# fluggo/Canvas

Hardware: AMD Instinct MI355X
Metric: Mpixels/s through 4K f16 RGBA colour-matrix+alpha-over chain; % HBM roofline (higher is better)
Workload: dtype f32

## Files before the change

### canvas_amd/csrc/host/color.c

```c
#include "internal.h"

CVS_EXPORT int cvs_color_matrix_f16_dev(rgba_frame_f16 *frame, const float m[9], int pre_lut, int post_lut, cvs_stream_t s) {
    if (cvs_enter() != 0) return -1;
    CVS_REQUIRE_INSIDE(frame, frame, "cvs_color_matrix_f16_dev");
    if (box2i_is_empty(&frame->current_window)) return 0;
    if (!cvs_box_contains(&frame->full_window, &frame->current_window)) { cvs_set_error("colour matrix: current_window outside the buffer"); return -1; }
    const half *pre = cvs_lut_dev_or_null(pre_lut), *post = cvs_lut_dev_or_null(post_lut);
    if ((pre_lut != CVS_LUT_NONE && !pre) || (post_lut != CVS_LUT_NONE && !post)) return -1;
    cvk_view v = cvs_view(frame->data, &frame->full_window);
    CVS_KERNEL(CVK(cvk_color_matrix)(v, v, cvs_rect(&frame->current_window), m, pre, post, cvs_cus(), cvs_pick_stream(s)));
    return 0;
}

CVS_EXPORT int cvs_color_matrix_f16_to_dev(rgba_frame_f16 *out, const rgba_frame_f16 *in, const float m[9], int pre_lut, int post_lut, cvs_stream_t s) {
    if (cvs_enter() != 0) { box2i_set_empty(&out->current_window); return -1; }
    CVS_REQUIRE_INSIDE(in, out, "cvs_color_matrix_f16_to_dev");
    box2i win;
    box2i_intersect(&win, &out->full_window, &in->current_window);
    out->current_window = win;
    if (box2i_is_empty(&win)) return 0;
    if (!cvs_box_contains(&in->full_window, &win)) { cvs_set_error("colour matrix: source window outside its buffer"); box2i_set_empty(&out->current_window); return -1; }
    const half *pre = cvs_lut_dev_or_null(pre_lut), *post = cvs_lut_dev_or_null(post_lut);
    if ((pre_lut != CVS_LUT_NONE && !pre) || (post_lut != CVS_LUT_NONE && !post)) { box2i_set_empty(&out->current_window); return -1; }
    CVS_KERNEL(CVK(cvk_color_matrix)(cvs_view(out->data, &out->full_window), cvs_view(in->data, &in->full_window), cvs_rect(&win), m, pre, post, cvs_cus(), cvs_pick_stream(s)));
    return 0;
}

static void host_color(rgba_frame_f16 *frame, const float m[9], int pre, int post) {
    if (box2i_is_empty(&frame->current_window) || cvs_enter() != 0) return;
    hipStream_t s = cvs_pick_stream(NULL);
    cvs_staged d = { 0 };
    rgba_frame_f16 f = *frame;
    int rc = cvs_stage_in(&d, frame->data, cvs_box_pixels(&frame->full_window) * sizeof(rgba_f16), 1, s);
    f.data = d.dev;
    if (rc == 0) rc = cvs_color_matrix_f16_dev(&f, m, pre, post, s);
    if (rc == 0) cvs_stage_out(&d, frame->data, s);
    cvs_stage_free(&d);
}

CVS_EXPORT void video_color_rgb_to_xyz_sdtv(rgba_frame_f16 *frame) {
    static const float m[9] = { 0.3936f, 0.2124f, 0.0187f, 0.3652f, 0.7010f, 0.1119f, 0.1916f, 0.0865f, 0.9582f };
    host_color(frame, m, CVS_LUT_REC709_TO_LINEAR_SCENE, CVS_LUT_NONE);
}

CVS_EXPORT void video_color_xyz_to_srgb(rgba_frame_f16 *frame) {
    static const float m[9] = { 3.2410f, -0.9692f, 0.0556f, -1.5374f, 1.8760f, -0.2040f, -0.4986f, 0.0416f, 1.0570f };
    host_color(frame, m, CVS_LUT_NONE, CVS_LUT_LINEAR_TO_SRGB);
}


static __thread int t_last_fused = -1;
CVS_EXPORT int cvs_chain_last_was_fused(void) { return t_last_fused; }
CVS_EXPORT int cvs_chain_last_launch_count(void) { return CVK(cvk_chain_count)(); }

static bool same_box(const box2i *a, const box2i *b) {
    return a->min.x == b->min.x && a->min.y == b->min.y && a->max.x == b->max.x && a->max.y == b->max.y;
}

static bool ranges_overlap(const void *a, const void *b, size_t bytes) {
    const uintptr_t x = (uintptr_t)a, y = (uintptr_t)b;
    return x < y + bytes && y < x + bytes;
}

static bool job_is_fusable(const cvs_chain_job *j) {
    if (j->nlayers < 1 || j->nlayers > CVS_CHAIN_MAX_LAYERS) return false;
    const box2i *fw = &j->out->full_window;
    if (box2i_is_empty(fw) || cvs_box_pixels(fw) < 2) return false;
    if (((uintptr_t)j->out->data & 15u) != 0) return false;
    const size_t bytes = cvs_box_pixels(fw) * sizeof(rgba_f16);
    for (int k = 0; k < j->nlayers; k++) {
        const rgba_frame_f16 *l = j->layers[k];
        if (!same_box(&l->full_window, fw) || !same_box(&l->current_window, fw)) return false;
        if (((uintptr_t)l->data & 15u) != 0) return false;
        if (l->data != j->out->data && ranges_overlap(l->data, j->out->data, bytes)) return false;
    }
    return true;
}

static bool job_depends_on_earlier(const cvs_chain_job *jobs, int first, int j) {
    const size_t bj = cvs_box_pixels(&jobs[j].out->full_window) * sizeof(rgba_f16);
    for (int i = first; i < j; i++) {
        const size_t bi = cvs_box_pixels(&jobs[i].out->full_window) * sizeof(rgba_f16);
        const size_t span = bi > bj ? bi : bj;
        if (ranges_overlap(jobs[j].out->data, jobs[i].out->data, span)) return true;
// ... 37 lines not shown

CVS_EXPORT int cvs_chain_color_over_f16_dev(const cvs_chain_job *jobs, int njobs, const float m[9],
                                            int pre_lut, int post_lut, cvs_stream_t stream) {
    if (cvs_enter() != 0) return -1;
    if (njobs <= 0) return 0;
    hipStream_t s = cvs_pick_stream(stream);
    if (!m && (pre_lut != CVS_LUT_NONE || post_lut != CVS_LUT_NONE)) { cvs_set_error("chain: transfer tables need a colour matrix (m == NULL means no colour stage)"); return -1; }
    const half *pre = cvs_lut_dev_or_null(pre_lut), *post = cvs_lut_dev_or_null(post_lut);
    if ((pre_lut != CVS_LUT_NONE && !pre) || (post_lut != CVS_LUT_NONE && !post)) return -1;

    bool all_fusable = true;
    for (int i = 0; i < njobs; i++) all_fusable = all_fusable && job_is_fusable(&jobs[i]);
    if (!all_fusable) {
        t_last_fused = 0;
        for (int i = 0; i < njobs; i++) {
            int rc = chain_unfused(&jobs[i], m, pre_lut, post_lut, s);
            if (rc != 0) return rc;
        }
        return 0;
    }

    cvk_chain_job *recs = calloc((size_t)njobs, sizeof *recs);
    if (!recs) { cvs_set_error("chain: out of host memory"); return -1; }
    int uniform = jobs[0].nlayers;
    for (int i = 0; i < njobs; i++) {
        cvk_chain_job *kj = &recs[i];
        kj->out = jobs[i].out->data;
        for (int k = 0; k < jobs[i].nlayers; k++) kj->layer[k] = jobs[i].layers[k]->data;
        kj->nlayers = jobs[i].nlayers;
        kj->npixels = cvs_box_pixels(&jobs[i].out->full_window);
        if (jobs[i].nlayers != uniform) uniform = 0;
        jobs[i].out->current_window = jobs[i].out->full_window;
    }
    int rc = 0;
    CVK(cvk_chain_count_reset)();
    for (int first = 0; rc == 0 && first < njobs; ) {
        int end = first + 1;
        while (end < njobs && !job_depends_on_earlier(jobs, first, end)) end++;
        rc = CVK(cvk_chain_color_over)(recs + first, end - first, uniform, m, pre, post, cvs_cus(), s);
        first = end;
    }
    free(recs);
    if (rc != 0) { cvs_set_error("chain kernel launch failed: %s", hipGetErrorString((hipError_t)rc)); return rc; }
    t_last_fused = 1;
    return 0;
}

CVS_EXPORT int cvs_mix_cross_f16_dev(rgba_frame_f16 *out, const rgba_frame_f16 *a, const rgba_frame_f16 *b, float mix_b, cvs_stream_t stream) {
    if (cvs_enter() != 0) { box2i_set_empty(&out->current_window); return -1; }
    CVS_REQUIRE_INSIDE(a, out, "cvs_mix_cross_f16_dev");
    CVS_REQUIRE_INSIDE(b, out, "cvs_mix_cross_f16_dev");
    hipStream_t s = cvs_pick_stream(stream);
    mix_b = clampf(mix_b, 0.0f, 1.0f);
    const cvs_chain_job job = { out, { a, b }, 2 };
    if (job_is_fusable(&job)) {
        cvk_chain_job rec;
        memset(&rec, 0, sizeof rec);
        rec.out = out->data; rec.layer[0] = a->data; rec.layer[1] = b->data; rec.nlayers = 2;
        rec.npixels = cvs_box_pixels(&out->full_window);
        int rc = CVK(cvk_chain_cross)(&rec, 1, 1.0f - mix_b, mix_b, cvs_cus(), s);
        if (rc != 0) { cvs_set_error("crossfade kernel launch failed: %s", hipGetErrorString((hipError_t)rc)); box2i_set_empty(&out->current_window); return rc; }
        out->current_window = out->full_window;
        t_last_fused = 1;
        return 0;
    }
    t_last_fused = 0;
    const box2i *fw = &out->full_window;
    const size_t n = cvs_box_pixels(fw);
    if (!n) { box2i_set_empty(&out->current_window); return 0; }
    rgba_frame_f32 fa = { cvs_pool_malloc(n * sizeof(rgba_f32), s), *fw, *fw }, fb = { cvs_pool_malloc(n * sizeof(rgba_f32), s), *fw, *fw };
    rgba_frame_f32 fo = { cvs_pool_malloc(n * sizeof(rgba_f32), s), *fw, *fw };
    int rc = (fa.data && fb.data && fo.data) ? 0 : -1;
    rgba_frame_f16 clip = { cvs_pool_malloc(n * sizeof(rgba_f16), s), *fw, *fw };
    if (!clip.data) rc = -1;
    if (rc == 0) rc = cvs_copy_frame_f16_dev(&clip, a, s);
    if (rc == 0) rc = cvs_frame_f16_to_f32_dev(&fa, &clip, s);
    if (rc == 0) rc = cvs_copy_frame_f16_dev(&clip, b, s);
    if (rc == 0) rc = cvs_frame_f16_to_f32_dev(&fb, &clip, s);
    if (rc == 0) rc = cvs_mix_cross_f32_dev(&fo, &fa, &fb, mix_b, s);
    if (rc == 0) rc = cvs_frame_f32_to_f16_dev(out, &fo, s);
    cvs_pool_free(clip.data, s); cvs_pool_free(fa.data, s); cvs_pool_free(fb.data, s); cvs_pool_free(fo.data, s);
    if (rc != 0) box2i_set_empty(&out->current_window);
    return rc;
}
```

### canvas_amd/csrc/kernels/chain_deep_ops.hip

```cpp
#include "chain_kernel.hpp"

namespace {

template <int NL, int DIAG>
int launch_mode(const BatchT<8> &b, int n, const Mat &mat, const uint16_t *pre, const uint16_t *post, unsigned grid, unsigned block, int lshift, hipStream_t s) {
    if (mat.plain) return launch<NL, CHAIN_PLAIN, DIAG>(b, n, mat, pre, post, grid, block, lshift, s);
    return launch<NL, CHAIN_GRADE, DIAG>(b, n, mat, pre, post, grid, block, lshift, s);
}

template <int DIAG>
int launch_deep(int nl, const BatchT<8> &b, int n, const Mat &mat, const uint16_t *pre, const uint16_t *post, unsigned grid, unsigned block, int lshift, hipStream_t s) {
    switch (nl) {
    case 5: return launch_mode<5, DIAG>(b, n, mat, pre, post, grid, block, lshift, s);
    case 6: return launch_mode<6, DIAG>(b, n, mat, pre, post, grid, block, lshift, s);
    case 7: return launch_mode<7, DIAG>(b, n, mat, pre, post, grid, block, lshift, s);
    default: return launch_mode<8, DIAG>(b, n, mat, pre, post, grid, block, lshift, s);
    }
}

}

extern "C" int cvk_chain_deep(const cvk_chain_job *jobs, int njobs, int nlayers, const cvs::Mat *mat, const uint16_t *pre, const uint16_t *post,
                              unsigned grid, unsigned block, int lshift, int diag, uint64_t bytes_per_launch, void *stream, int *taken) {
    if (nlayers < 5 || nlayers > 8 || mat->cross || block > 512) return (int)hipErrorInvalidValue;
    BatchT<8> b;
    const int n = fill_batch(b, jobs, njobs, nlayers, bytes_per_launch);
    *taken = n;
    hipStream_t s = (hipStream_t)stream;
#ifdef CVS_DIAG
    if (diag == DIAG_MEMORY_ONLY) return launch_deep<DIAG_MEMORY_ONLY>(nlayers, b, n, *mat, pre, post, grid, block, lshift, s);
    if (diag == DIAG_COMPUTE_ONLY) return launch_deep<DIAG_COMPUTE_ONLY>(nlayers, b, n, *mat, pre, post, grid, block, lshift, s);
#endif
    (void)diag;
    return launch_deep<DIAG_NONE>(nlayers, b, n, *mat, pre, post, grid, block, lshift, s);
}
```

### canvas_amd/csrc/kernels/chain_kernel.hpp

```cpp
#pragma once
#include "lut_common.hpp"
#include "grade.hpp"
#include "chain_math.hpp"
#include <string.h>

namespace {

using namespace cvs;

template <int ML> struct JobCT { void *out; const void *layer[ML]; uint64_t npixels; };
template <int ML> struct BatchT {
    static constexpr int kJobs = ML == 4 ? 64 : 48;
    JobCT<ML> jobs[kJobs];
};
template <int ML>
inline int fill_batch(BatchT<ML> &b, const cvk_chain_job *jobs, int njobs, int nlayers, uint64_t bytes_per_launch) {
    memset(&b, 0, sizeof b);
    uint64_t bytes = 0;
    int n = 0;
    while (n < njobs && n < BatchT<ML>::kJobs) {
        const cvk_chain_job &src = jobs[n];
        const uint64_t job_bytes = src.npixels * 8 * (uint64_t)(nlayers + 1);
        if (n > 0 && bytes + job_bytes > bytes_per_launch) break;
        b.jobs[n].out = src.out;
// ... 36 lines not shown

__device__ __forceinline__ void stage_lut_any(uint16_t *lds, const uint16_t *__restrict__ table) {
    const uint4 *src = reinterpret_cast<const uint4 *>(table);
    uint4 *dst = reinterpret_cast<uint4 *>(lds);
    constexpr int kWords = kLutHalfs * 2 / 16;
    if (kWords % blockDim.x == 0) {
        const int slices = kWords / (int)blockDim.x, rot = (int)(blockIdx.x >> 3);
        for (int it = 0; it < slices; it++) {
            const int i = ((it + rot) % slices) * (int)blockDim.x + (int)threadIdx.x;
            dst[i] = src[i];
        }
    } else {
        for (int i = threadIdx.x; i < kWords; i += blockDim.x) dst[i] = src[i];
    }
    __syncthreads();
}

enum { DIAG_NONE = 0, DIAG_MEMORY_ONLY = 1, DIAG_COMPUTE_ONLY = 2 };

template <int NL>
struct Walk {
    unsigned job;
    unsigned chunk;
    unsigned npairs;
    unsigned nchunks;
    const char *layer[NL];
    char *out;
};

constexpr bool chain_hand_pipelined(int nl, int mode, bool pre, bool post) {
    return !(nl == 6 && mode == CHAIN_GRADE && pre && !post);
}

template <int NL, int MODE, bool PRE, bool POST, int DIAG>
__global__ __launch_bounds__(NL <= 4 ? kWG : 512) void k_chain(BatchT<(NL <= 4 ? 4 : 8)> batch, int njobs_, Mat kmat, int lshift,
                                               const uint16_t *__restrict__ pre, const uint16_t *__restrict__ post) {
    constexpr bool HAND = chain_hand_pipelined(NL, MODE, PRE, POST);
    const MatR mat = CVS_MAT_REGS(kmat);
    __shared__ uint16_t lut[(PRE || POST) ? kLutHalfs : 1];
    const unsigned L = 1u << lshift, G = gridDim.x, tid = threadIdx.x, njobs = (unsigned)njobs_;

    auto load_job = [&](Walk<NL> &w) {
        const auto &job = batch.jobs[w.job];
        w.npairs = (unsigned)(job.npixels >> 1);
        w.nchunks = (w.npairs + L - 1) >> lshift;
#pragma unroll
        for (int k = 0; k < NL; k++) w.layer[k] = reinterpret_cast<const char *>(job.layer[k]);
        w.out = reinterpret_cast<char *>(job.out);
    };
    auto advance = [&](Walk<NL> &w, unsigned by) {
        w.chunk += by;
        while (w.chunk >= w.nchunks) {
            w.chunk -= w.nchunks;
            if (++w.job >= njobs) { w.job = njobs; w.chunk = 0; return; }
            load_job(w);
        }
    };
    auto valid_of = [&](const Walk<NL> &w) -> unsigned { const unsigned left = w.npairs - (w.chunk << lshift); return left < L ? left : L; };
    auto issue = [&](u32x4 (&dst)[NL], const Walk<NL> &w) {
        const unsigned valid = valid_of(w);
        const uint32_t voff = (tid < valid ? tid : valid - 1) << 4;
#pragma unroll
        for (int k = 0; k < NL; k++) {
            const char *base = w.layer[k] + ((size_t)w.chunk << (lshift + 4));
            if constexpr (HAND) asm_ld4s(dst[k], base, voff);
            else dst[k] = __builtin_nontemporal_load(reinterpret_cast<const u32x4 *>(base + voff));
        }
    };

    Walk<NL> cur;
    cur.job = 0; cur.chunk = 0;
    load_job(cur);
    advance(cur, blockIdx.x);
    if (cur.job >= njobs) return;
    Walk<NL> next = cur;
    advance(next, G);

    u32x4 A[NL], B[NL];
    u32x4 diag_acc = { 0, 0, 0, 0 };
    issue(A, cur);
    if (PRE) stage_lut_any(lut, pre);
    else if (POST) stage_lut_any(lut, post);
    if constexpr (HAND) wait_vm0(A);
    if (next.job < njobs) issue(B, next);

    auto trip = [&](u32x4 (&now)[NL], u32x4 (&nxt)[NL]) -> bool {
        u32x4 res;
        if (DIAG == DIAG_MEMORY_ONLY) {
            res = now[0];
#pragma unroll
            for (int k = 1; k < NL; k++) res ^= now[k];
        } else {
            res = chain_pair_lean<NL, PRE, POST, MODE>(now, mat, lut, post);
        }
        Walk<NL> after = next;
        if (after.job < njobs) advance(after, G);
        const bool store_it = tid < valid_of(cur);
        g_u4 out = (g_u4)(cur.out + ((size_t)cur.chunk << (lshift + 4)));
        __builtin_amdgcn_sched_barrier(0);
        if constexpr (HAND) wait_vm0(nxt);
        __builtin_amdgcn_sched_barrier(0);
        if (DIAG == DIAG_COMPUTE_ONLY) diag_acc ^= res;
        else if (store_it) __builtin_nontemporal_store(res, out + tid);
        if (after.job < njobs) {
            if (DIAG == DIAG_COMPUTE_ONLY) {
#pragma unroll
                for (int k = 0; k < NL; k++) now[k] = nxt[k];
            } else {
                issue(now, after);
            }
        }
        __builtin_amdgcn_sched_barrier(0);
        cur = next;
        next = after;
        return cur.job < njobs;
    };
    while (trip(A, B) && trip(B, A)) { }
    if (DIAG == DIAG_COMPUTE_ONLY) ((g_u4)batch.jobs[0].out)[(size_t)blockIdx.x * L + tid] = diag_acc;

}

template <int NL, int MODE, bool PRE, bool POST>
__global__ __launch_bounds__(64) void k_chain_tail(BatchT<(NL <= 4 ? 4 : 8)> batch, int njobs, Mat kmat, const uint16_t *__restrict__ pre, const uint16_t *__restrict__ post) {
    MatR mat = CVS_MAT_REGS(kmat);
    mat.plain = MODE == CHAIN_PLAIN; mat.cross = MODE == CHAIN_CROSS;
    const int j = (int)threadIdx.x;
    if (j >= njobs) return;
    const auto &job = batch.jobs[j];
    if (!(job.npixels & 1)) return;
    uint2 px[NL];
#pragma unroll
    for (int k = 0; k < NL; k++) px[k] = ld2(job.layer[k], job.npixels - 1);
    st2(job.out, job.npixels - 1, chain_pixel<NL, PRE, POST>(px, NL, mat, PRE ? pre : post, post));
}

template <int NL, int MODE, int DIAG>
int launch(const BatchT<(NL <= 4 ? 4 : 8)> &jobs, int njobs, const Mat &mat, const uint16_t *pre, const uint16_t *post, unsigned grid, unsigned block, int lshift, hipStream_t s) {
    bool odd = false;
    for (int i = 0; i < njobs; i++) odd = odd || (jobs.jobs[i].npixels & 1);
    if constexpr (MODE != CHAIN_GRADE) {
        hipLaunchKernelGGL((k_chain<NL, MODE, false, false, DIAG>), dim3(grid), dim3(block), 0, s, jobs, njobs, mat, lshift, pre, post);
        if (odd) hipLaunchKernelGGL((k_chain_tail<NL, MODE, false, false>), dim3(1), dim3(64), 0, s, jobs, njobs, mat, pre, post);
    } else {
        if (pre && post)  hipLaunchKernelGGL((k_chain<NL, MODE, true, true, DIAG>), dim3(grid), dim3(block), 0, s, jobs, njobs, mat, lshift, pre, post);
        else if (pre)     hipLaunchKernelGGL((k_chain<NL, MODE, true, false, DIAG>), dim3(grid), dim3(block), 0, s, jobs, njobs, mat, lshift, pre, post);
        else if (post)    hipLaunchKernelGGL((k_chain<NL, MODE, false, true, DIAG>), dim3(grid), dim3(block), 0, s, jobs, njobs, mat, lshift, pre, post);
        else              hipLaunchKernelGGL((k_chain<NL, MODE, false, false, DIAG>), dim3(grid), dim3(block), 0, s, jobs, njobs, mat, lshift, pre, post);
        if (odd) {
            if (pre && post)  hipLaunchKernelGGL((k_chain_tail<NL, MODE, true, true>), dim3(1), dim3(64), 0, s, jobs, njobs, mat, pre, post);
            else if (pre)     hipLaunchKernelGGL((k_chain_tail<NL, MODE, true, false>), dim3(1), dim3(64), 0, s, jobs, njobs, mat, pre, post);
            else if (post)    hipLaunchKernelGGL((k_chain_tail<NL, MODE, false, true>), dim3(1), dim3(64), 0, s, jobs, njobs, mat, pre, post);
            else              hipLaunchKernelGGL((k_chain_tail<NL, MODE, false, false>), dim3(1), dim3(64), 0, s, jobs, njobs, mat, pre, post);
        }
    }
    return (int)hipGetLastError();
}


}
```

### canvas_amd/csrc/kernels/chain_ops.hip

```cpp
#include "chain_kernel.hpp"
#include <stdlib.h>

extern "C" int cvk_chain_deep(const cvk_chain_job *jobs, int njobs, int nlayers, const cvs::Mat *mat, const uint16_t *pre, const uint16_t *post,
                              unsigned grid, unsigned block, int lshift, int diag, uint64_t bytes_per_launch, void *stream, int *taken);

namespace {

#ifdef CVS_CONTRACT
constexpr int kJobsPerLaunchV0 = 32, kFusedLayers = 4;
#else
constexpr int kJobsPerLaunchV0 = 32, kFusedLayers = 8;
#endif
typedef BatchT<4> Batch;
constexpr uint64_t kBytesPerLaunch = 8ull * 3840 * 2160 * 24;
constexpr int kChainBlock = 512, kChainBlockLog2 = 9;
struct BatchV0 { cvk_chain_job jobs[kJobsPerLaunchV0]; };


template <int NL, bool PRE, bool POST>
__global__ __launch_bounds__(kWG) void k_chain_v0(BatchV0 batch, int njobs, Mat kmat,
                                                  const uint16_t *__restrict__ pre, const uint16_t *__restrict__ post) {
    const MatR mat = CVS_MAT_REGS(kmat);
    __shared__ uint16_t lut[(PRE || POST) ? kLutHalfs : 1];
    if (PRE) stage_lut(lut, pre);
    else if (POST) stage_lut(lut, post);
    constexpr int MAXL = NL > 0 ? NL : CVK_CHAIN_MAX_LAYERS;
    const size_t stride = (size_t)gridDim.x * kWG;
    for (int j = 0; j < njobs; j++) {
        const cvk_chain_job &job = batch.jobs[j];
        const int nl = NL > 0 ? NL : job.nlayers;
        const size_t npairs = job.npixels / 2;
        for (size_t i = (size_t)blockIdx.x * kWG + threadIdx.x; i < npairs; i += stride) {
            uint4 a[MAXL];
#pragma unroll
            for (int k = 0; k < MAXL; k++) if (k < nl) a[k] = ld4(job.layer[k], i);
            uint2 p0[MAXL], p1[MAXL];
#pragma unroll
            for (int k = 0; k < MAXL; k++) { p0[k] = make_uint2(a[k].x, a[k].y); p1[k] = make_uint2(a[k].z, a[k].w); }
            uint2 r0 = chain_pixel<MAXL, PRE, POST>(p0, nl, mat, lut, post), r1 = chain_pixel<MAXL, PRE, POST>(p1, nl, mat, lut, post);
            st4(job.out, i, make_uint4(r0.x, r0.y, r1.x, r1.y));
        }
        if ((job.npixels & 1) && blockIdx.x == 0 && threadIdx.x == 0) {
            uint2 p[MAXL];
#pragma unroll
            for (int k = 0; k < MAXL; k++) if (k < nl) p[k] = ld2(job.layer[k], job.npixels - 1);
            st2(job.out, job.npixels - 1, chain_pixel<MAXL, PRE, POST>(p, nl, mat, lut, post));
        }
    }
}

template <int DIAG>
int launch_nl(int nl, const Batch &b, int n, const Mat &mat, const uint16_t *pre, const uint16_t *post, unsigned grid, unsigned block, int lshift, hipStream_t s) {
    if (mat.cross) return launch<2, CHAIN_CROSS, DIAG>(b, n, mat, pre, post, grid, block, lshift, s);
    if (mat.plain) {
        switch (nl) {
        case 1: return launch<1, CHAIN_PLAIN, DIAG>(b, n, mat, pre, post, grid, block, lshift, s);
        case 2: return launch<2, CHAIN_PLAIN, DIAG>(b, n, mat, pre, post, grid, block, lshift, s);
        case 3: return launch<3, CHAIN_PLAIN, DIAG>(b, n, mat, pre, post, grid, block, lshift, s);
        default: return launch<4, CHAIN_PLAIN, DIAG>(b, n, mat, pre, post, grid, block, lshift, s);
        }
    }
    switch (nl) {
    case 1: return launch<1, CHAIN_GRADE, DIAG>(b, n, mat, pre, post, grid, block, lshift, s);
    case 2: return launch<2, CHAIN_GRADE, DIAG>(b, n, mat, pre, post, grid, block, lshift, s);
    case 3: return launch<3, CHAIN_GRADE, DIAG>(b, n, mat, pre, post, grid, block, lshift, s);
    default: return launch<4, CHAIN_GRADE, DIAG>(b, n, mat, pre, post, grid, block, lshift, s);
    }
}

template <int NL>
int launch_v0(const BatchV0 &jobs, int njobs, const Mat &mat, const uint16_t *pre, const uint16_t *post, unsigned grid, hipStream_t s) {
    if (pre && post)  hipLaunchKernelGGL((k_chain_v0<NL, true, true>), dim3(grid), dim3(kWG), 0, s, jobs, njobs, mat, pre, post);
    else if (pre)     hipLaunchKernelGGL((k_chain_v0<NL, true, false>), dim3(grid), dim3(kWG), 0, s, jobs, njobs, mat, pre, post);
    else if (post)    hipLaunchKernelGGL((k_chain_v0<NL, false, true>), dim3(grid), dim3(kWG), 0, s, jobs, njobs, mat, pre, post);
    else              hipLaunchKernelGGL((k_chain_v0<NL, false, false>), dim3(grid), dim3(kWG), 0, s, jobs, njobs, mat, pre, post);
    return (int)hipGetLastError();
}

struct Tuning { int variant; unsigned block; int lshift; uint64_t bytes_per_launch; };

Tuning tuning() {
    Tuning t = { 1, (unsigned)kChainBlock, kChainBlockLog2, kBytesPerLaunch };
#ifdef CVS_DIAG
    if (const char *e = getenv("CVS_CHAIN_VARIANT")) t.variant = atoi(e);
    if (const char *e = getenv("CVS_CHAIN_BLOCK")) {
        const int b = atoi(e);
        if (b == 256) { t.block = 256; t.lshift = 8; } else if (b == 1024) { t.block = 1024; t.lshift = 10; }
    }
    if (const char *e = getenv("CVS_CHAIN_LAUNCH_MB")) { const long long mb = atoll(e); if (mb > 0) t.bytes_per_launch = (uint64_t)mb << 20; }
#endif
    return t;
}

thread_local int t_launches = 0;

int chain_dispatch(const cvk_chain_job *jobs, int njobs, int uniform_layers, const Mat &mat,
                   const uint16_t *pre, const uint16_t *post, int cus, void *stream) {
    const unsigned grid = (unsigned)(cus > 0 ? cus : 256);
    hipStream_t s = (hipStream_t)stream;
    const Tuning t = tuning();
    bool fused_kernel = t.variant != 0 && uniform_layers >= 1 && uniform_layers <= kFusedLayers;
    for (int i = 0; fused_kernel && i < njobs; i++)
        if (jobs[i].npixels < 2 || jobs[i].npixels * 8 >= (1ull << 32)) fused_kernel = false;
    int first = 0;
    while (first < njobs) {
        int n = 0, rc;
#ifndef CVS_CONTRACT
        if (fused_kernel && uniform_layers > 4) {
            const int diag = t.variant == 10 ? DIAG_MEMORY_ONLY : t.variant == 12 ? DIAG_COMPUTE_ONLY : DIAG_NONE;
            rc = cvk_chain_deep(jobs + first, njobs - first, uniform_layers, &mat, pre, post, grid, t.block, t.lshift, diag, t.bytes_per_launch, stream, &n);
        } else
#endif
        if (fused_kernel) {
            Batch b;
            n = fill_batch(b, jobs + first, njobs - first, uniform_layers, t.bytes_per_launch);
#ifdef CVS_DIAG
            if (t.variant == 10) rc = launch_nl<DIAG_MEMORY_ONLY>(uniform_layers, b, n, mat, pre, post, grid, t.block, t.lshift, s);
            else if (t.variant == 12) rc = launch_nl<DIAG_COMPUTE_ONLY>(uniform_layers, b, n, mat, pre, post, grid, t.block, t.lshift, s);
            else
#endif
            rc = launch_nl<DIAG_NONE>(uniform_layers, b, n, mat, pre, post, grid, t.block, t.lshift, s);
        } else {
            BatchV0 b;
            memset(&b, 0, sizeof b);
            n = njobs - first < kJobsPerLaunchV0 ? njobs - first : kJobsPerLaunchV0;
            memcpy(b.jobs, jobs + first, sizeof(cvk_chain_job) * (size_t)n);
            switch (uniform_layers) {
            case 1: rc = launch_v0<1>(b, n, mat, pre, post, grid, s); break;
            case 2: rc = launch_v0<2>(b, n, mat, pre, post, grid, s); break;
            case 3: rc = launch_v0<3>(b, n, mat, pre, post, grid, s); break;
            case 4: rc = launch_v0<4>(b, n, mat, pre, post, grid, s); break;
            default: rc = launch_v0<0>(b, n, mat, pre, post, grid, s); break;
            }
        }
        if (rc != 0) return rc;
        first += n;
        t_launches++;
    }
    return 0;
}

}

extern "C" void cvk_chain_count_reset(void) { t_launches = 0; }
extern "C" int cvk_chain_count(void) { return t_launches; }

extern "C" int cvk_chain_color_over(const cvk_chain_job *jobs, int njobs, int uniform_layers, const float *m,
                                    const uint16_t *pre, const uint16_t *post, int cus, void *stream) {
    return chain_dispatch(jobs, njobs, uniform_layers, make_mat(m), pre, post, cus, stream);
}

extern "C" int cvk_chain_cross(const cvk_chain_job *jobs, int njobs, float wa, float wb, int cus, void *stream) {
    Mat mat = make_mat(NULL);
    mat.plain = 0; mat.cross = 1; mat.wa = wa; mat.wb = wb;
    return chain_dispatch(jobs, njobs, 2, mat, NULL, NULL, cus, stream);
}
```

### canvas_amd/csrc/kernels/kernels.h

```cpp
#ifndef CVS_KERNELS_H
#define CVS_KERNELS_H

#include <stddef.h>
#include <stdint.h>

#ifdef CVS_DIAG
#include <stdlib.h>
#define CVS_DIAG_ENV(name) getenv(name)
#else
#define CVS_DIAG_ENV(name) ((const char *)0)
#endif

#ifdef CVS_CONTRACT
#define cvk_gain_offset_f16          cvk_gain_offset_f16_fma
#define cvk_mix                      cvk_mix_fma
#define cvk_color_matrix             cvk_color_matrix_fma
#define cvk_chain_color_over         cvk_chain_color_over_fma
#define cvk_chain_cross              cvk_chain_cross_fma
#define cvk_chain_count_reset        cvk_chain_count_reset_fma
#define cvk_chain_count              cvk_chain_count_fma
#define cvk_fir_gather               cvk_fir_gather_fma
#define cvk_fir2d_lds_bytes          cvk_fir2d_lds_bytes_fma
#define cvk_fir2d                    cvk_fir2d_fma
#define cvk_fir_vh_supported         cvk_fir_vh_supported_fma
// ... 35 lines not shown
int cvk_copy_alpha_f32(cvk_view out, cvk_view in, cvk_rect r, float alpha, void *stream);
int cvk_weave_f16(cvk_view frame, cvk_rect cur, const void *other, cvk_rect other_cur, void *stream);
int cvk_widen(cvk_view out32, cvk_view in16, cvk_rect r, void *stream);
int cvk_narrow(cvk_view out16, cvk_view in32, cvk_rect r, void *stream);
int cvk_fill_f16(cvk_view out, cvk_rect r, const float rgba[4], void *stream);
int cvk_fill_f32(cvk_view out, cvk_rect r, const float rgba[4], void *stream);
int cvk_gain_offset_f16(cvk_view out, cvk_view in, cvk_rect r, float gain, float offset, void *stream);

enum { CVK_MIX_CROSS = 0, CVK_MIX_OVER = 1 };
typedef struct {
    cvk_view out, p, q;
    cvk_rect outer, inner;
    cvk_rect pw, qw;
    int gap_x, gap_y;
    int top_is_p, bottom_is_p, left_is_p, right_is_p;
    float wp, wq;
    int mode;
    int p_in_place;
} cvk_mix_params;
int cvk_mix(const cvk_mix_params *mp, void *stream);

int cvk_color_matrix(cvk_view dst, cvk_view src, cvk_rect r, const float m[9], const uint16_t *pre_lut,
                     const uint16_t *post_lut, int cus, void *stream);

#define CVK_CHAIN_MAX_LAYERS 8
typedef struct {
    void *out;
    const void *layer[CVK_CHAIN_MAX_LAYERS];
    int nlayers;
    int pad;
    uint64_t npixels;
} cvk_chain_job;
int cvk_chain_color_over(const cvk_chain_job *jobs, int njobs, int uniform_layers, const float *m,
                         const uint16_t *pre_lut, const uint16_t *post_lut, int cus, void *stream);

void cvk_chain_count_reset(void);
int cvk_chain_count(void);

int cvk_chain_cross(const cvk_chain_job *jobs, int njobs, float wa, float wb, int cus, void *stream);

typedef struct {
    cvk_view target, source;
    int axis;
    int t0, t1;
    int lo, hi;
    int s0, s1;
    const int *ntaps;
    const int *tap_src;
    const float *taps;
    int stride;
    int in_half, out_half;
} cvk_fir_params;
int cvk_fir_gather(const cvk_fir_params *fp, void *stream);
int cvk_zero_f32(cvk_view v, void *stream);

typedef struct {
    const int *ntaps, *src;
    const float *taps;
    const int *foot;
    int stride;
    int lines;
    int max_taps;
    int wide_foot;
    int max_active;
    int streamable;
    const uint32_t *lrec;
    const uint32_t *pack;
    int pack_width;
    int span_lines[3];
} cvk_fir_axis;
#define CVK_FIR_LREC 32
#define CVK_AXIS_ALIGN(bytes)              (((size_t)(bytes) + 255) & ~(size_t)255)
// ... 56 lines not shown
int cvk_blur_pair(const cvk_blur_params *bp, int cus, void *stream);

typedef struct {
    cvk_view target, source;
    int in_half, out_half;
    int tx0, ty0, tx1, ty1;
    int sx0, sy0, sx1, sy1;
    int ntaps1, ntaps2;
    int rows_per_wg;
    int flags;
    float taps1[16], taps2[16];
    cvk_frame_batch batch;
} cvk_blur_halve_params;
int cvk_blur_halve_supported(int ntaps1, int ntaps2);
int cvk_blur_halve_pair_supported(const cvk_blur_halve_params *bp);
int cvk_blur_halve_pair(const cvk_blur_halve_params *bp, int cus, void *stream);
int cvk_blur_halve_takes_pairs(const cvk_blur_halve_params *bp);
int cvk_blur_halve(const cvk_blur_halve_params *bp, int cus, void *stream);

enum { CVK_DISPLAY_RGBA8 = 0, CVK_DISPLAY_ARGB32_PREMUL = 1 };
int cvk_display(void *dst, cvk_view src, cvk_rect r, const uint8_t *table, int mode, int cus, void *stream);

typedef struct { uint8_t *y, *cb, *cr; int sy, scb, scr; } cvk_dv_planes;
typedef struct { float coeff[16]; int width, center; } cvk_dv_taps;
int cvk_dv_reconstruct(cvk_view frame, cvk_rect cur, const cvk_dv_planes *pl, const cvk_dv_taps *tri, const uint16_t *lut, void *stream);
int cvk_dv_subsample(const cvk_dv_planes *pl, cvk_view frame, cvk_rect w, const cvk_dv_taps *tri, const uint16_t *lut, int encode_in_place, void *stream);

int cvk_mpeg2_subsample(const cvk_dv_planes *pl, cvk_view frame, cvk_rect w, int width, int height, const uint16_t *lut, int cus, void *stream);

#ifndef CVS_CONTRACT
int cvk_gain_offset_f16_fma(cvk_view out, cvk_view in, cvk_rect r, float gain, float offset, void *stream);
int cvk_mix_fma(const cvk_mix_params *mp, void *stream);
int cvk_color_matrix_fma(cvk_view dst, cvk_view src, cvk_rect r, const float m[9], const uint16_t *pre_lut, const uint16_t *post_lut, int cus, void *stream);
int cvk_chain_color_over_fma(const cvk_chain_job *jobs, int njobs, int uniform_layers, const float *m, const uint16_t *pre_lut, const uint16_t *post_lut, int cus, void *stream);
int cvk_chain_cross_fma(const cvk_chain_job *jobs, int njobs, float wa, float wb, int cus, void *stream);
void cvk_chain_count_reset_fma(void);
int cvk_chain_count_fma(void);
int cvk_fir_gather_fma(const cvk_fir_params *fp, void *stream);
size_t cvk_fir2d_lds_bytes_fma(const cvk_fir2d_params *fp);
int cvk_fir2d_fma(const cvk_fir2d_params *fp, void *stream);
int cvk_fir_vh_supported_fma(const cvk_fir2d_params *fp);
int cvk_fir_vh_fma(const cvk_fir2d_params *fp, int line0, int cus, void *stream);
int cvk_fir_tvh_supported_fma(const cvk_fir2d_params *fp);
int cvk_fir_tvh_preferred_fma(const cvk_fir2d_params *fp);
int cvk_fir_tvh_fma(const cvk_fir2d_params *fp, int line0, void *stream);
int cvk_blur_supported_fma(int ntaps, int step);
int cvk_blur_takes_pairs_fma(const cvk_blur_params *bp);
int cvk_blur_fma(const cvk_blur_params *bp, int cus, void *stream);
int cvk_blur_pair_supported_fma(const cvk_blur_params *bp);
int cvk_blur_pair_fma(const cvk_blur_params *bp, int cus, void *stream);
int cvk_blur_halve_pair_supported_fma(const cvk_blur_halve_params *bp);
int cvk_blur_halve_pair_fma(const cvk_blur_halve_params *bp, int cus, void *stream);
int cvk_blur_halve_supported_fma(int ntaps1, int ntaps2);
int cvk_blur_halve_takes_pairs_fma(const cvk_blur_halve_params *bp);
int cvk_blur_halve_fma(const cvk_blur_halve_params *bp, int cus, void *stream);
int cvk_dv_reconstruct_fma(cvk_view frame, cvk_rect cur, const cvk_dv_planes *pl, const cvk_dv_taps *tri, const uint16_t *lut, void *stream);
int cvk_dv_subsample_fma(const cvk_dv_planes *pl, cvk_view frame, cvk_rect w, const cvk_dv_taps *tri, const uint16_t *lut, int encode_in_place, void *stream);
#endif

#ifdef __cplusplus
}
#endif
#endif
```

Before: 258,300.

## Add atomic-ticket dynamic work distribution with strided runs to fused chain kernel

Replaces the static grid-stride chunk assignment in the fused colour-over chain kernel (for up to 4 layers) with dynamic scheduling. Blocks draw tickets from a global atomic counter, each ticket covering a run of chunks, and the draw is prefetched one run ahead and handed through LDS. Each launch now covers the whole batch instead of being split by bytes-per-launch. The goal is to even out load across CUs and cut tail imbalance and per-launch overhead. The cost is a pool allocation and a memset of the ticket counter per call, an LDS barrier per run, and hand-written exec-mask asm that is fragile.

```diff
diff --git a/canvas_amd/csrc/host/color.c b/canvas_amd/csrc/host/color.c
--- a/canvas_amd/csrc/host/color.c
+++ b/canvas_amd/csrc/host/color.c
@@ -50,6 +50,7 @@
 
 
 static __thread int t_last_fused = -1;
+static const size_t kTicketBytes = 256;
 CVS_EXPORT int cvs_chain_last_was_fused(void) { return t_last_fused; }
 CVS_EXPORT int cvs_chain_last_launch_count(void) { return CVK(cvk_chain_count)(); }
 
@@ -153,14 +154,17 @@
         if (jobs[i].nlayers != uniform) uniform = 0;
         jobs[i].out->current_window = jobs[i].out->full_window;
     }
+    unsigned *tickets = cvs_pool_malloc(kTicketBytes, s);
+    if (!tickets) { free(recs); return -1; }
     int rc = 0;
     CVK(cvk_chain_count_reset)();
     for (int first = 0; rc == 0 && first < njobs; ) {
         int end = first + 1;
         while (end < njobs && !job_depends_on_earlier(jobs, first, end)) end++;
-        rc = CVK(cvk_chain_color_over)(recs + first, end - first, uniform, m, pre, post, cvs_cus(), s);
+        rc = CVK(cvk_chain_color_over)(recs + first, end - first, uniform, m, pre, post, cvs_cus(), tickets, s);
         first = end;
     }
+    cvs_pool_free(tickets, s);
     free(recs);
     if (rc != 0) { cvs_set_error("chain kernel launch failed: %s", hipGetErrorString((hipError_t)rc)); return rc; }
     t_last_fused = 1;
@@ -179,7 +183,10 @@
         memset(&rec, 0, sizeof rec);
         rec.out = out->data; rec.layer[0] = a->data; rec.layer[1] = b->data; rec.nlayers = 2;
         rec.npixels = cvs_box_pixels(&out->full_window);
-        int rc = CVK(cvk_chain_cross)(&rec, 1, 1.0f - mix_b, mix_b, cvs_cus(), s);
+        unsigned *tickets = cvs_pool_malloc(kTicketBytes, s);
+        if (!tickets) { box2i_set_empty(&out->current_window); return -1; }
+        int rc = CVK(cvk_chain_cross)(&rec, 1, 1.0f - mix_b, mix_b, cvs_cus(), tickets, s);
+        cvs_pool_free(tickets, s);
         if (rc != 0) { cvs_set_error("crossfade kernel launch failed: %s", hipGetErrorString((hipError_t)rc)); box2i_set_empty(&out->current_window); return rc; }
         out->current_window = out->full_window;
         t_last_fused = 1;
diff --git a/canvas_amd/csrc/kernels/chain_deep_ops.hip b/canvas_amd/csrc/kernels/chain_deep_ops.hip
--- a/canvas_amd/csrc/kernels/chain_deep_ops.hip
+++ b/canvas_amd/csrc/kernels/chain_deep_ops.hip
@@ -3,34 +3,36 @@
 namespace {
 
 template <int NL, int DIAG>
-int launch_mode(const BatchT<8> &b, int n, const Mat &mat, const uint16_t *pre, const uint16_t *post, unsigned grid, unsigned block, int lshift, hipStream_t s) {
-    if (mat.plain) return launch<NL, CHAIN_PLAIN, DIAG>(b, n, mat, pre, post, grid, block, lshift, s);
-    return launch<NL, CHAIN_GRADE, DIAG>(b, n, mat, pre, post, grid, block, lshift, s);
+int launch_mode(const BatchT<8> &b, int n, const Mat &mat, const uint16_t *pre, const uint16_t *post, unsigned grid, unsigned block, int lshift, const Sched &sc, hipStream_t s) {
+    if (mat.plain) return launch<NL, CHAIN_PLAIN, DIAG>(b, n, mat, pre, post, grid, block, lshift, sc, s);
+    return launch<NL, CHAIN_GRADE, DIAG>(b, n, mat, pre, post, grid, block, lshift, sc, s);
 }
 
 template <int DIAG>
-int launch_deep(int nl, const BatchT<8> &b, int n, const Mat &mat, const uint16_t *pre, const uint16_t *post, unsigned grid, unsigned block, int lshift, hipStream_t s) {
+int launch_deep(int nl, const BatchT<8> &b, int n, const Mat &mat, const uint16_t *pre, const uint16_t *post, unsigned grid, unsigned block, int lshift, const Sched &sc, hipStream_t s) {
     switch (nl) {
-    case 5: return launch_mode<5, DIAG>(b, n, mat, pre, post, grid, block, lshift, s);
-    case 6: return launch_mode<6, DIAG>(b, n, mat, pre, post, grid, block, lshift, s);
-    case 7: return launch_mode<7, DIAG>(b, n, mat, pre, post, grid, block, lshift, s);
-    default: return launch_mode<8, DIAG>(b, n, mat, pre, post, grid, block, lshift, s);
+    case 5: return launch_mode<5, DIAG>(b, n, mat, pre, post, grid, block, lshift, sc, s);
+    case 6: return launch_mode<6, DIAG>(b, n, mat, pre, post, grid, block, lshift, sc, s);
+    case 7: return launch_mode<7, DIAG>(b, n, mat, pre, post, grid, block, lshift, sc, s);
+    default: return launch_mode<8, DIAG>(b, n, mat, pre, post, grid, block, lshift, sc, s);
     }
 }
 
 }
 
 extern "C" int cvk_chain_deep(const cvk_chain_job *jobs, int njobs, int nlayers, const cvs::Mat *mat, const uint16_t *pre, const uint16_t *post,
-                              unsigned grid, unsigned block, int lshift, int diag, uint64_t bytes_per_launch, void *stream, int *taken) {
+                              unsigned grid, unsigned block, int lshift, int diag, uint64_t bytes_per_launch, unsigned *tickets, int run, int strided,
+                              void *stream, int *taken) {
     if (nlayers < 5 || nlayers > 8 || mat->cross || block > 512) return (int)hipErrorInvalidValue;
     BatchT<8> b;
     const int n = fill_batch(b, jobs, njobs, nlayers, bytes_per_launch);
     *taken = n;
     hipStream_t s = (hipStream_t)stream;
+    const Sched sc = { tickets, run, strided };
 #ifdef CVS_DIAG
-    if (diag == DIAG_MEMORY_ONLY) return launch_deep<DIAG_MEMORY_ONLY>(nlayers, b, n, *mat, pre, post, grid, block, lshift, s);
-    if (diag == DIAG_COMPUTE_ONLY) return launch_deep<DIAG_COMPUTE_ONLY>(nlayers, b, n, *mat, pre, post, grid, block, lshift, s);
+    if (diag == DIAG_MEMORY_ONLY) return launch_deep<DIAG_MEMORY_ONLY>(nlayers, b, n, *mat, pre, post, grid, block, lshift, sc, s);
+    if (diag == DIAG_COMPUTE_ONLY) return launch_deep<DIAG_COMPUTE_ONLY>(nlayers, b, n, *mat, pre, post, grid, block, lshift, sc, s);
 #endif
     (void)diag;
-    return launch_deep<DIAG_NONE>(nlayers, b, n, *mat, pre, post, grid, block, lshift, s);
+    return launch_deep<DIAG_NONE>(nlayers, b, n, *mat, pre, post, grid, block, lshift, sc, s);
 }
diff --git a/canvas_amd/csrc/kernels/chain_kernel.hpp b/canvas_amd/csrc/kernels/chain_kernel.hpp
--- a/canvas_amd/csrc/kernels/chain_kernel.hpp
+++ b/canvas_amd/csrc/kernels/chain_kernel.hpp
@@ -92,13 +92,40 @@
     return !(nl == 6 && mode == CHAIN_GRADE && pre && !post);
 }
 
+__device__ __forceinline__ void asm_ticket(unsigned &dst, unsigned *ctr, unsigned one) {
+    uint64_t saved;
+    asm volatile("s_mov_b64 %1, exec\n\t"
+                 "s_mov_b32 exec_lo, %3\n\t"
+                 "s_mov_b32 exec_hi, 0\n\t"
+                 "global_atomic_add %0, %4, %5, %2 sc0\n\t"
+                 "s_mov_b64 exec, %1"
+                 : "=&v"(dst), "=&s"(saved) : "s"(ctr), "s"(__builtin_amdgcn_readfirstlane(one)), "v"(0u), "v"(1u) : "memory");
+}
+
+constexpr int kRunTrips = 8;
+constexpr bool kRunStrided = true;
+
+__device__ __forceinline__ void lds_barrier() { asm volatile("s_waitcnt lgkmcnt(0)\n\ts_barrier" : : : "memory"); }
+
 template <int NL, int MODE, bool PRE, bool POST, int DIAG>
 __global__ __launch_bounds__(NL <= 4 ? kWG : 512) void k_chain(BatchT<(NL <= 4 ? 4 : 8)> batch, int njobs_, Mat kmat, int lshift,
-                                               const uint16_t *__restrict__ pre, const uint16_t *__restrict__ post) {
+                                               const uint16_t *__restrict__ pre, const uint16_t *__restrict__ post,
+                                               unsigned *__restrict__ tickets, int run_, int strided_) {
     constexpr bool HAND = chain_hand_pipelined(NL, MODE, PRE, POST);
     const MatR mat = CVS_MAT_REGS(kmat);
     __shared__ uint16_t lut[(PRE || POST) ? kLutHalfs : 1];
+    __shared__ unsigned ticket_ring[2];
     const unsigned L = 1u << lshift, G = gridDim.x, tid = threadIdx.x, njobs = (unsigned)njobs_;
+#ifdef CVS_DIAG
+    const bool ticketed = NL <= 4 && tickets != nullptr, strided = strided_ != 0;
+    const unsigned S = (unsigned)run_;
+#else
+    constexpr bool ticketed = NL <= 4, strided = kRunStrided;
+    constexpr unsigned S = kRunTrips;
+    (void)run_; (void)strided_;
+#endif
+    const unsigned step = strided ? G : 1u;
+    auto start_of = [&](unsigned t) -> unsigned { return strided ? (t / G) * G * S + t % G : t * S; };
 
     auto load_job = [&](Walk<NL> &w) {
         const auto &job = batch.jobs[w.job];
@@ -131,10 +158,41 @@
     Walk<NL> cur;
     cur.job = 0; cur.chunk = 0;
     load_job(cur);
-    advance(cur, blockIdx.x);
+    advance(cur, ticketed ? start_of(blockIdx.x) : blockIdx.x);
     if (cur.job >= njobs) return;
+    unsigned rs_job = cur.job, rs_chunk = cur.chunk;
+    unsigned rs_at = ticketed ? start_of(blockIdx.x) : blockIdx.x, k = 0, tk = G + blockIdx.x, nev = 0, pend = 0;
+    const unsigned drawer = __builtin_amdgcn_readfirstlane(tid == 0 ? 1u : 0u);
+    if (ticketed) asm_ticket(pend, tickets, drawer);
+    auto step_from = [&](Walk<NL> &w) -> bool {
+        if (w.job >= njobs) return false;
+        if (!ticketed) { advance(w, G); return false; }
+        if (k + 1 < S) {
+            advance(w, step);
+            k++;
+            if (w.job < njobs) return false;
+        }
+        const unsigned at = start_of(tk);
+        w.job = rs_job; w.chunk = rs_chunk;
+        load_job(w);
+        advance(w, at - rs_at);
+        rs_job = w.job; rs_chunk = w.chunk; rs_at = at; k = 0;
+        return w.job < njobs;
+    };
+    auto publish = [&]() { if (tid == 0) ticket_ring[nev & 1] = pend; };
+    auto take = [&]() {
+        if (!ticketed) return;
+        lds_barrier();
+        tk = __builtin_amdgcn_readfirstlane(ticket_ring[nev & 1]) + 2 * G;
+        asm_ticket(pend, tickets, drawer);
+        nev++;
+    };
     Walk<NL> next = cur;
-    advance(next, G);
+    if (step_from(next)) {
+        asm volatile("s_waitcnt vmcnt(0)" : "+v"(pend) : : "memory");
+        publish();
+        take();
+    }
 
     u32x4 A[NL], B[NL];
     u32x4 diag_acc = { 0, 0, 0, 0 };
@@ -154,12 +212,13 @@
             res = chain_pair_lean<NL, PRE, POST, MODE>(now, mat, lut, post);
         }
         Walk<NL> after = next;
-        if (after.job < njobs) advance(after, G);
+        const bool run_started = step_from(after);
         const bool store_it = tid < valid_of(cur);
         g_u4 out = (g_u4)(cur.out + ((size_t)cur.chunk << (lshift + 4)));
         __builtin_amdgcn_sched_barrier(0);
         if constexpr (HAND) wait_vm0(nxt);
         __builtin_amdgcn_sched_barrier(0);
+        if (run_started) publish();
         if (DIAG == DIAG_COMPUTE_ONLY) diag_acc ^= res;
         else if (store_it) __builtin_nontemporal_store(res, out + tid);
         if (after.job < njobs) {
@@ -171,6 +230,10 @@
             }
         }
         __builtin_amdgcn_sched_barrier(0);
+        if (run_started) {
+            take();
+            __builtin_amdgcn_sched_barrier(0);
+        }
         cur = next;
         next = after;
         return cur.job < njobs;
@@ -194,18 +257,25 @@
     st2(job.out, job.npixels - 1, chain_pixel<NL, PRE, POST>(px, NL, mat, PRE ? pre : post, post));
 }
 
+struct Sched { unsigned *tickets; int run; int strided; };
+
 template <int NL, int MODE, int DIAG>
-int launch(const BatchT<(NL <= 4 ? 4 : 8)> &jobs, int njobs, const Mat &mat, const uint16_t *pre, const uint16_t *post, unsigned grid, unsigned block, int lshift, hipStream_t s) {
+int launch(const BatchT<(NL <= 4 ? 4 : 8)> &jobs, int njobs, const Mat &mat, const uint16_t *pre, const uint16_t *post, unsigned grid, unsigned block, int lshift,
+           const Sched &sc, hipStream_t s) {
     bool odd = false;
     for (int i = 0; i < njobs; i++) odd = odd || (jobs.jobs[i].npixels & 1);
+    if (sc.tickets) {
+        const hipError_t e = hipMemsetAsync(sc.tickets, 0, sizeof(unsigned), s);
+        if (e != hipSuccess) return (int)e;
+    }
     if constexpr (MODE != CHAIN_GRADE) {
-        hipLaunchKernelGGL((k_chain<NL, MODE, false, false, DIAG>), dim3(grid), dim3(block), 0, s, jobs, njobs, mat, lshift, pre, post);
+        hipLaunchKernelGGL((k_chain<NL, MODE, false, false, DIAG>), dim3(grid), dim3(block), 0, s, jobs, njobs, mat, lshift, pre, post, sc.tickets, sc.run, sc.strided);
         if (odd) hipLaunchKernelGGL((k_chain_tail<NL, MODE, false, false>), dim3(1), dim3(64), 0, s, jobs, njobs, mat, pre, post);
     } else {
-        if (pre && post)  hipLaunchKernelGGL((k_chain<NL, MODE, true, true, DIAG>), dim3(grid), dim3(block), 0, s, jobs, njobs, mat, lshift, pre, post);
-        else if (pre)     hipLaunchKernelGGL((k_chain<NL, MODE, true, false, DIAG>), dim3(grid), dim3(block), 0, s, jobs, njobs, mat, lshift, pre, post);
-        else if (post)    hipLaunchKernelGGL((k_chain<NL, MODE, false, true, DIAG>), dim3(grid), dim3(block), 0, s, jobs, njobs, mat, lshift, pre, post);
-        else              hipLaunchKernelGGL((k_chain<NL, MODE, false, false, DIAG>), dim3(grid), dim3(block), 0, s, jobs, njobs, mat, lshift, pre, post);
+        if (pre && post)  hipLaunchKernelGGL((k_chain<NL, MODE, true, true, DIAG>), dim3(grid), dim3(block), 0, s, jobs, njobs, mat, lshift, pre, post, sc.tickets, sc.run, sc.strided);
+        else if (pre)     hipLaunchKernelGGL((k_chain<NL, MODE, true, false, DIAG>), dim3(grid), dim3(block), 0, s, jobs, njobs, mat, lshift, pre, post, sc.tickets, sc.run, sc.strided);
+        else if (post)    hipLaunchKernelGGL((k_chain<NL, MODE, false, true, DIAG>), dim3(grid), dim3(block), 0, s, jobs, njobs, mat, lshift, pre, post, sc.tickets, sc.run, sc.strided);
+        else              hipLaunchKernelGGL((k_chain<NL, MODE, false, false, DIAG>), dim3(grid), dim3(block), 0, s, jobs, njobs, mat, lshift, pre, post, sc.tickets, sc.run, sc.strided);
         if (odd) {
             if (pre && post)  hipLaunchKernelGGL((k_chain_tail<NL, MODE, true, true>), dim3(1), dim3(64), 0, s, jobs, njobs, mat, pre, post);
             else if (pre)     hipLaunchKernelGGL((k_chain_tail<NL, MODE, true, false>), dim3(1), dim3(64), 0, s, jobs, njobs, mat, pre, post);
diff --git a/canvas_amd/csrc/kernels/chain_ops.hip b/canvas_amd/csrc/kernels/chain_ops.hip
--- a/canvas_amd/csrc/kernels/chain_ops.hip
+++ b/canvas_amd/csrc/kernels/chain_ops.hip
@@ -2,7 +2,8 @@
 #include <stdlib.h>
 
 extern "C" int cvk_chain_deep(const cvk_chain_job *jobs, int njobs, int nlayers, const cvs::Mat *mat, const uint16_t *pre, const uint16_t *post,
-                              unsigned grid, unsigned block, int lshift, int diag, uint64_t bytes_per_launch, void *stream, int *taken);
+                              unsigned grid, unsigned block, int lshift, int diag, uint64_t bytes_per_launch, unsigned *tickets, int run, int strided,
+                              void *stream, int *taken);
 
 namespace {
 
@@ -50,21 +51,21 @@
 }
 
 template <int DIAG>
-int launch_nl(int nl, const Batch &b, int n, const Mat &mat, const uint16_t *pre, const uint16_t *post, unsigned grid, unsigned block, int lshift, hipStream_t s) {
-    if (mat.cross) return launch<2, CHAIN_CROSS, DIAG>(b, n, mat, pre, post, grid, block, lshift, s);
+int launch_nl(int nl, const Batch &b, int n, const Mat &mat, const uint16_t *pre, const uint16_t *post, unsigned grid, unsigned block, int lshift, const Sched &sc, hipStream_t s) {
+    if (mat.cross) return launch<2, CHAIN_CROSS, DIAG>(b, n, mat, pre, post, grid, block, lshift, sc, s);
     if (mat.plain) {
         switch (nl) {
-        case 1: return launch<1, CHAIN_PLAIN, DIAG>(b, n, mat, pre, post, grid, block, lshift, s);
-        case 2: return launch<2, CHAIN_PLAIN, DIAG>(b, n, mat, pre, post, grid, block, lshift, s);
-        case 3: return launch<3, CHAIN_PLAIN, DIAG>(b, n, mat, pre, post, grid, block, lshift, s);
-        default: return launch<4, CHAIN_PLAIN, DIAG>(b, n, mat, pre, post, grid, block, lshift, s);
+        case 1: return launch<1, CHAIN_PLAIN, DIAG>(b, n, mat, pre, post, grid, block, lshift, sc, s);
+        case 2: return launch<2, CHAIN_PLAIN, DIAG>(b, n, mat, pre, post, grid, block, lshift, sc, s);
+        case 3: return launch<3, CHAIN_PLAIN, DIAG>(b, n, mat, pre, post, grid, block, lshift, sc, s);
+        default: return launch<4, CHAIN_PLAIN, DIAG>(b, n, mat, pre, post, grid, block, lshift, sc, s);
         }
     }
     switch (nl) {
-    case 1: return launch<1, CHAIN_GRADE, DIAG>(b, n, mat, pre, post, grid, block, lshift, s);
-    case 2: return launch<2, CHAIN_GRADE, DIAG>(b, n, mat, pre, post, grid, block, lshift, s);
-    case 3: return launch<3, CHAIN_GRADE, DIAG>(b, n, mat, pre, post, grid, block, lshift, s);
-    default: return launch<4, CHAIN_GRADE, DIAG>(b, n, mat, pre, post, grid, block, lshift, s);
+    case 1: return launch<1, CHAIN_GRADE, DIAG>(b, n, mat, pre, post, grid, block, lshift, sc, s);
+    case 2: return launch<2, CHAIN_GRADE, DIAG>(b, n, mat, pre, post, grid, block, lshift, sc, s);
+    case 3: return launch<3, CHAIN_GRADE, DIAG>(b, n, mat, pre, post, grid, block, lshift, sc, s);
+    default: return launch<4, CHAIN_GRADE, DIAG>(b, n, mat, pre, post, grid, block, lshift, sc, s);
     }
 }
 
@@ -77,10 +78,10 @@
     return (int)hipGetLastError();
 }
 
-struct Tuning { int variant; unsigned block; int lshift; uint64_t bytes_per_launch; };
+struct Tuning { int variant; unsigned block; int lshift; uint64_t bytes_per_launch; int run; int strided; };
 
 Tuning tuning() {
-    Tuning t = { 1, (unsigned)kChainBlock, kChainBlockLog2, kBytesPerLaunch };
+    Tuning t = { 1, (unsigned)kChainBlock, kChainBlockLog2, kBytesPerLaunch, kRunTrips, kRunStrided ? 1 : 0 };
 #ifdef CVS_DIAG
     if (const char *e = getenv("CVS_CHAIN_VARIANT")) t.variant = atoi(e);
     if (const char *e = getenv("CVS_CHAIN_BLOCK")) {
@@ -88,6 +89,8 @@
         if (b == 256) { t.block = 256; t.lshift = 8; } else if (b == 1024) { t.block = 1024; t.lshift = 10; }
     }
     if (const char *e = getenv("CVS_CHAIN_LAUNCH_MB")) { const long long mb = atoll(e); if (mb > 0) t.bytes_per_launch = (uint64_t)mb << 20; }
+    if (const char *e = getenv("CVS_CHAIN_RUN")) { const int r = atoi(e); if (r >= 1 && r <= 64) t.run = r; }
+    if (const char *e = getenv("CVS_CHAIN_STRIDED")) t.strided = atoi(e) != 0;
 #endif
     return t;
 }
@@ -95,10 +98,14 @@
 thread_local int t_launches = 0;
 
 int chain_dispatch(const cvk_chain_job *jobs, int njobs, int uniform_layers, const Mat &mat,
-                   const uint16_t *pre, const uint16_t *post, int cus, void *stream) {
+                   const uint16_t *pre, const uint16_t *post, int cus, unsigned *tickets, void *stream) {
     const unsigned grid = (unsigned)(cus > 0 ? cus : 256);
     hipStream_t s = (hipStream_t)stream;
     const Tuning t = tuning();
+    if (t.variant == 2) tickets = nullptr;
+    else if (!tickets) return (int)hipErrorInvalidValue;
+    const Sched sc = { tickets, t.run, t.strided };
+    const uint64_t bytes_per_launch = tickets ? ~0ull : t.bytes_per_launch;
     bool fused_kernel = t.variant != 0 && uniform_layers >= 1 && uniform_layers <= kFusedLayers;
     for (int i = 0; fused_kernel && i < njobs; i++)
         if (jobs[i].npixels < 2 || jobs[i].npixels * 8 >= (1ull << 32)) fused_kernel = false;
@@ -108,18 +115,18 @@
 #ifndef CVS_CONTRACT
         if (fused_kernel && uniform_layers > 4) {
             const int diag = t.variant == 10 ? DIAG_MEMORY_ONLY : t.variant == 12 ? DIAG_COMPUTE_ONLY : DIAG_NONE;
-            rc = cvk_chain_deep(jobs + first, njobs - first, uniform_layers, &mat, pre, post, grid, t.block, t.lshift, diag, t.bytes_per_launch, stream, &n);
+            rc = cvk_chain_deep(jobs + first, njobs - first, uniform_layers, &mat, pre, post, grid, t.block, t.lshift, diag, t.bytes_per_launch, nullptr, 0, 0, stream, &n);
         } else
 #endif
         if (fused_kernel) {
             Batch b;
-            n = fill_batch(b, jobs + first, njobs - first, uniform_layers, t.bytes_per_launch);
+            n = fill_batch(b, jobs + first, njobs - first, uniform_layers, bytes_per_launch);
 #ifdef CVS_DIAG
-            if (t.variant == 10) rc = launch_nl<DIAG_MEMORY_ONLY>(uniform_layers, b, n, mat, pre, post, grid, t.block, t.lshift, s);
-            else if (t.variant == 12) rc = launch_nl<DIAG_COMPUTE_ONLY>(uniform_layers, b, n, mat, pre, post, grid, t.block, t.lshift, s);
+            if (t.variant == 10) rc = launch_nl<DIAG_MEMORY_ONLY>(uniform_layers, b, n, mat, pre, post, grid, t.block, t.lshift, sc, s);
+            else if (t.variant == 12) rc = launch_nl<DIAG_COMPUTE_ONLY>(uniform_layers, b, n, mat, pre, post, grid, t.block, t.lshift, sc, s);
             else
 #endif
-            rc = launch_nl<DIAG_NONE>(uniform_layers, b, n, mat, pre, post, grid, t.block, t.lshift, s);
+            rc = launch_nl<DIAG_NONE>(uniform_layers, b, n, mat, pre, post, grid, t.block, t.lshift, sc, s);
         } else {
             BatchV0 b;
             memset(&b, 0, sizeof b);
@@ -146,12 +153,12 @@
 extern "C" int cvk_chain_count(void) { return t_launches; }
 
 extern "C" int cvk_chain_color_over(const cvk_chain_job *jobs, int njobs, int uniform_layers, const float *m,
-                                    const uint16_t *pre, const uint16_t *post, int cus, void *stream) {
-    return chain_dispatch(jobs, njobs, uniform_layers, make_mat(m), pre, post, cus, stream);
+                                    const uint16_t *pre, const uint16_t *post, int cus, unsigned *tickets, void *stream) {
+    return chain_dispatch(jobs, njobs, uniform_layers, make_mat(m), pre, post, cus, tickets, stream);
 }
 
-extern "C" int cvk_chain_cross(const cvk_chain_job *jobs, int njobs, float wa, float wb, int cus, void *stream) {
+extern "C" int cvk_chain_cross(const cvk_chain_job *jobs, int njobs, float wa, float wb, int cus, unsigned *tickets, void *stream) {
     Mat mat = make_mat(NULL);
     mat.plain = 0; mat.cross = 1; mat.wa = wa; mat.wb = wb;
-    return chain_dispatch(jobs, njobs, 2, mat, NULL, NULL, cus, stream);
+    return chain_dispatch(jobs, njobs, 2, mat, NULL, NULL, cus, tickets, stream);
 }
diff --git a/canvas_amd/csrc/kernels/kernels.h b/canvas_amd/csrc/kernels/kernels.h
--- a/canvas_amd/csrc/kernels/kernels.h
+++ b/canvas_amd/csrc/kernels/kernels.h
@@ -91,12 +91,12 @@
     uint64_t npixels;
 } cvk_chain_job;
 int cvk_chain_color_over(const cvk_chain_job *jobs, int njobs, int uniform_layers, const float *m,
-                         const uint16_t *pre_lut, const uint16_t *post_lut, int cus, void *stream);
+                         const uint16_t *pre_lut, const uint16_t *post_lut, int cus, unsigned *tickets, void *stream);
 
 void cvk_chain_count_reset(void);
 int cvk_chain_count(void);
 
-int cvk_chain_cross(const cvk_chain_job *jobs, int njobs, float wa, float wb, int cus, void *stream);
+int cvk_chain_cross(const cvk_chain_job *jobs, int njobs, float wa, float wb, int cus, unsigned *tickets, void *stream);
 
 typedef struct {
     cvk_view target, source;
@@ -219,8 +219,8 @@
 int cvk_gain_offset_f16_fma(cvk_view out, cvk_view in, cvk_rect r, float gain, float offset, void *stream);
 int cvk_mix_fma(const cvk_mix_params *mp, void *stream);
 int cvk_color_matrix_fma(cvk_view dst, cvk_view src, cvk_rect r, const float m[9], const uint16_t *pre_lut, const uint16_t *post_lut, int cus, void *stream);
-int cvk_chain_color_over_fma(const cvk_chain_job *jobs, int njobs, int uniform_layers, const float *m, const uint16_t *pre_lut, const uint16_t *post_lut, int cus, void *stream);
-int cvk_chain_cross_fma(const cvk_chain_job *jobs, int njobs, float wa, float wb, int cus, void *stream);
+int cvk_chain_color_over_fma(const cvk_chain_job *jobs, int njobs, int uniform_layers, const float *m, const uint16_t *pre_lut, const uint16_t *post_lut, int cus, unsigned *tickets, void *stream);
+int cvk_chain_cross_fma(const cvk_chain_job *jobs, int njobs, float wa, float wb, int cus, unsigned *tickets, void *stream);
 void cvk_chain_count_reset_fma(void);
 int cvk_chain_count_fma(void);
 int cvk_fir_gather_fma(const cvk_fir_params *fp, void *stream);
```

Result: slower. 255,500, median of 6 (-1.1%).
